# gsw4869/CUDA_LDPC

Measured on AMD Instinct MI355X. Metric: decoded codewords/sec (50-iter flooding min-sum, fixed iterations), higher is better.
Workload: dtype f32; 1 GPU; J4_L24_Z96 rate-0.833 batch=65536 codewords/GPU 50 iters Es/N0=3.0dB; kernel=qc_lds_halfrow-local<nf2,J4,L24,Z96,wc20,wv4,g4,w6>t768_lds79904, frames_per_gpu=65536

## Files before the change

### cuda_ldpc_amd/csrc/bldpc_qc2_body.inc

```
template <typename GM, bool HIST> __global__ __launch_bounds__(GM::TPB, GM::MINW) void QC2_NAME(QcArgs a)
{
    constexpr int NF = GM::NF, L = GM::L, Z = GM::Z, WC = GM::WC, WV = GM::WV, GJ = GM::GJ, ZB = GM::ZB, WCH = GM::WCH;
    constexpr int RPT = GM::RPT, CPT = GM::CPT, NCG = GM::NCG, MSG = GM::MSG;
    static_assert(NF == 2, "the half-row kernel carries a frame pair per lane");
    constexpr bool LOC = GM::LOC;
    constexpr int NL = LOC ? CPT : 0;
    extern __shared__ __attribute__((aligned(16))) char lds[];
    const int chunk = (a.nWG + 7) >> 3;
#if QC2_PERSIST
    const int xcd = (int)(blockIdx.x & 7);
    int wg = 0;
#else
    const int wg = (int)(blockIdx.x & 7) * chunk + (int)(blockIdx.x >> 3);
    if (wg >= a.nWG) return;
#endif

    const int F = a.F;
    const int tid = threadIdx.x;
    const int wave = tid >> 6, lane = tid & 63, h = lane >> 5;
    const int jq = wave / ZB, t = (wave - jq * ZB) * 32 + (lane & 31);
    const int cg = jq * 2 + h;
#if QC2_PERSIST
    int f0 = 0;
#else
    const int f0 = wg * NF;
#endif
    int *lds_flag = reinterpret_cast<int *>(lds + GM::flag_byte);

    const int rbase = ((jq * WC + h * WCH) * Z + t) * MSG;
    const int sbase = (GM::Sslot + cg * Z + t) * MSG;
    int saddr[RPT][WCH];
    v2f32 Rr[RPT][WCH];
    int e0v[RPT], wrv[RPT];
#pragma unroll
    for (int rr = 0; rr < RPT; rr++) {
        e0v[rr] = a.rowptr[jq + rr * GJ];
        wrv[rr] = a.rowptr[jq + rr * GJ + 1] - e0v[rr];
    }
    int wcv[CPT];
#pragma unroll
    for (int cc = 0; cc < CPT; cc++) wcv[cc] = LOC ? 0 : a.wv[cg + cc * NCG];
    int sst[LOC ? CPT : 1];
    int cl[LOC ? CPT : 1];
#pragma unroll
    for (int rr = 0; rr < RPT; rr++) {
        QcCnEdge ed[WCH];
#pragma unroll
        for (int i = 0; i < WCH; i++) ed[i] = a.cn_edges[e0v[rr] + min(h * WCH + i, wrv[rr] - 1)];
#pragma unroll
        for (int i = 0; i < WCH; i++) {
            int c = t + ed[i].shift;
            c = (c >= Z) ? c - Z : c;
            const int slot = (h * WCH + i < wrv[rr]) ? GM::Sslot + ed[i].col * Z + c : GM::inf_slot;
            saddr[rr][i] = slot * MSG;
            if constexpr (LOC) {
                if (i < NL) {
                    sst[i] = slot * MSG;
                    cl[i] = c;
                }
            }
#if !QC2_PERSIST
            Rr[rr][i] = v2f32{0.0f, 0.0f};
            lds_st2(rbase + (rr * GJ * WC + i) * Z * MSG, Rr[rr][i]);
#endif
        }
    }
    v2f32 yreg[CPT];
    int raddr[CPT][WV];
    auto y_load = [&](int cc) -> v2f32 {
        const int n = LOC ? sst[LOC ? cc : 0] / MSG - GM::Sslot : (cg + cc * NCG) * Z + t;
        return a.y_raw ? *reinterpret_cast<const v2f32 *>(a.y_raw + (size_t)n * F + f0)
                       : *reinterpret_cast<const v2f32 *>(a.y + ((size_t)wg * (L * Z) + n) * NF);
    };
#pragma unroll
    for (int cc = 0; cc < CPT; cc++) {
        const int l = cg + cc * NCG;
        if constexpr (LOC) {
            QcVnEdge ed[WV - 1];
#pragma unroll
            for (int kk = 0; kk < WV - 1; kk++) ed[kk] = a.vn_edges[l * WV + kk + (kk >= jq ? 1 : 0)];
#if !QC2_PERSIST
            yreg[cc] = y_load(cc);
#endif
#pragma unroll
            for (int kk = 0; kk < WV - 1; kk++) {
                int r = cl[cc] - ed[kk].shift;
                r = (r < 0) ? r + Z : r;
                raddr[cc][kk] = ((ed[kk].e != 0xffffu) ? ed[kk].e * Z + r : GM::zero_slot) * MSG;
            }
        } else {
        QcVnEdge ed[WV];
#pragma unroll
        for (int k = 0; k < WV; k++) ed[k] = a.vn_edges[l * WV + min(k, wcv[cc] - 1)];
#if !QC2_PERSIST
        yreg[cc] = y_load(cc);
#endif
#pragma unroll
        for (int k = 0; k < WV; k++) {
            int r = t - ed[k].shift;
            r = (r < 0) ? r + Z : r;
            raddr[cc][k] = ((k < wcv[cc]) ? ed[k].e * Z + r : GM::zero_slot) * MSG;
        }
        }
    }
    if (tid < NF) {
        reinterpret_cast<float *>(lds)[GM::zero_slot * NF + tid] = 0.0f;
        reinterpret_cast<float *>(lds)[GM::inf_slot * NF + tid] = __builtin_inff();
        lds_flag[tid] = 0;
        lds_flag[NF + tid] = 0;
    }
    unsigned long long hist = 0;
    unsigned done = 0;
    constexpr unsigned ALL = (1u << NF) - 1u;
#ifdef QC_STAMPS
    int nst = 0;
    auto stamp = [&](unsigned long long v) { if (tid == 0 && nst < QC_STAMPS) a.stamps[(size_t)wg * QC_STAMPS + nst++] = v; };
    const unsigned hwid = __builtin_amdgcn_s_getreg((31 << 11) | 4), xcc = __builtin_amdgcn_s_getreg((31 << 11) | 20);
    stamp(((unsigned long long)xcc << 32) | hwid);
    stamp(__builtin_amdgcn_s_memtime());
    if (a.stagger && ((hwid >> 16) & 1))
        for (int i = 0; i < a.stagger; i += 64 * 16) __builtin_amdgcn_s_sleep(16);
#endif
#if !QC2_PERSIST
    __syncthreads();
#endif
#ifdef QC_STAMPS
    stamp(__builtin_amdgcn_s_memtime());
#endif

    auto vn_phase = [&](bool (&bad)[NF]) {
        constexpr int CB = (CPT * WV <= 12) ? CPT : 1;
        static_for<CPT / CB>([&](auto C0) {
            constexpr int c0 = decltype(C0)::value * CB;
            v2f32 R[CB][WV];
#pragma unroll
            for (int ci = 0; ci < CB; ci++)
#pragma unroll
                for (int k = 0; k < WV; k++) R[ci][k] = lds_ld2(raddr[c0 + ci][k]);
            static_for<CB>([&](auto CI) {
                constexpr int ci = decltype(CI)::value, cc = c0 + ci;
                v2f32 S = v2f32{0.0f, 0.0f};
#pragma unroll
                for (int k = 0; k < WV; k++) S = S + R[ci][k];
                S = S + yreg[cc];
                lds_st2_imm<cc * NCG * Z * MSG>(sbase, S);
                if (HIST) {
                    const bool in_len = ((cg + cc * NCG) * Z + t) < a.length;
                    bad[0] = bad[0] || (in_len && S.x < 0);
                    bad[1] = bad[1] || (in_len && S.y < 0);
                }
            });
            if (CB < CPT) __builtin_amdgcn_sched_barrier(0);
        });
        asm volatile("s_waitcnt lgkmcnt(0)" ::: "memory");
    };
    v2f32 Sloc[LOC ? CPT : 1];
    const int jqs = __builtin_amdgcn_readfirstlane(jq);
    auto vn_phase_loc = [&](auto JJ, bool (&bad)[NF]) {
        constexpr int jj = decltype(JJ)::value;
        v2f32 R[CPT][WV - 1];
#pragma unroll
        for (int cc = 0; cc < CPT; cc++)
#pragma unroll
            for (int kk = 0; kk < WV - 1; kk++) R[cc][kk] = lds_ld2(raddr[cc][kk]);
        static_for<CPT>([&](auto CC) {
            constexpr int cc = decltype(CC)::value;
            v2f32 S = v2f32{0.0f, 0.0f};
            static_for<WV>([&](auto K) {
                constexpr int k = decltype(K)::value;
                if constexpr (k == jj) S = S + Rr[0][cc];
                else S = S + R[cc][k - (k > jj ? 1 : 0)];
            });
            S = S + yreg[cc];
            Sloc[LOC ? cc : 0] = S;
            lds_st2_imm<0>(sst[LOC ? cc : 0], S);
            if (HIST) {
                const bool in_len = (sst[LOC ? cc : 0] / MSG - GM::Sslot) < a.length;
                bad[0] = bad[0] || (in_len && S.x < 0);
                bad[1] = bad[1] || (in_len && S.y < 0);
            }
        });
        asm volatile("s_waitcnt lgkmcnt(0)" ::: "memory");
    };
    auto vn_any = [&](bool (&bad)[NF]) {
        if constexpr (LOC) static_for<GM::J>([&](auto JJ) { if (jqs == decltype(JJ)::value) vn_phase_loc(JJ, bad); });
        else vn_phase(bad);
    };
    auto flags_publish = [&](const bool (&bad)[NF], int it) {
#pragma unroll
        for (int v = 0; v < NF; v++)
            if (bad[v]) lds_flag[(it & 1) * NF + v] = 1;
    };
    auto flags_collect = [&](int it) -> int {
        int flag = 0;
        if (tid < NF) {
            flag = lds_flag[(it & 1) * NF + tid] ? 0 : 1;
            lds_flag[((it + 1) & 1) * NF + tid] = 0;
            if (flag && it <= 64) hist |= (1ull << (it - 1));
        }
        return flag;
    };
    auto emit = [&](unsigned mask, bool (&bad)[NF]) {
        unsigned *obits = a.bits;
        float *oapp = a.app;
        asm volatile("" : "+s"(obits), "+s"(oapp));
#pragma unroll
        for (int cc = 0; cc < CPT; cc++) {
            const int n = (cg + cc * NCG) * Z + t;
            float S[NF];
            lds_ld<NF>(S, lds, sbase + cc * NCG * Z * MSG);
#pragma unroll
            for (int v = 0; v < NF; v++) {
                if (HIST && !((mask >> v) & 1u)) continue;
                const bool neg = S[v] < 0;
                if (!HIST) bad[v] = bad[v] || (n < a.length && neg);
                const unsigned long long m = __ballot(neg);
                if ((tid & 31) == 0 && f0 + v < F) obits[(size_t)(f0 + v) * GM::NW + (n >> 5)] = (unsigned)(m >> (tid & 32));
                if (oapp && f0 + v < F) oapp[(size_t)n * F + f0 + v] = S[v];
            }
        }
    };
    auto retire = [&](int it) -> bool {
        unsigned newly = 0;
#pragma unroll
        for (int v = 0; v < NF; v++)
            if (!lds_flag[(it & 1) * NF + v]) newly |= 1u << v;
        newly &= ~done;
        if (newly) {
            bool unused[NF];
            emit(newly, unused);
            if (tid < NF && ((newly >> tid) & 1u) && f0 + tid < F) a.iters[f0 + tid] = it;
            done |= newly;
        }
        return done == ALL;
    };

#if QC2_PERSIST
    for (;;) {
    if (tid == 0) lds_flag[0] = atomicAdd(&a.work[xcd], 1);
    __syncthreads();
    {
        const int ord = __builtin_amdgcn_readfirstlane(lds_flag[0]);
        if (ord >= chunk || xcd * chunk + ord >= a.nWG) break;
        wg = xcd * chunk + ord;
    }
    __syncthreads();
    f0 = wg * NF;
#pragma unroll
    for (int rr = 0; rr < RPT; rr++)
#pragma unroll
        for (int i = 0; i < WCH; i++) {
            Rr[rr][i] = v2f32{0.0f, 0.0f};
            lds_st2(rbase + (rr * GJ * WC + i) * Z * MSG, Rr[rr][i]);
        }
#pragma unroll
    for (int cc = 0; cc < CPT; cc++) {
        yreg[cc] = y_load(cc);
    }
    if (tid < NF) {
        lds_flag[tid] = 0;
        lds_flag[NF + tid] = 0;
    }
    hist = 0;
    done = 0;
    __syncthreads();
#endif
    auto iterate = [&](auto JJ) {
    for (int it = 1; it < a.max_iter; it++) {
        bool bad[NF];
#pragma unroll
        for (int v = 0; v < NF; v++) bad[v] = false;
        __builtin_amdgcn_s_setprio(QC_PRIO_VN);
        if constexpr (LOC) vn_phase_loc(JJ, bad);
        else vn_phase(bad);
        if (HIST) flags_publish(bad, it);
        __syncthreads();
        __builtin_amdgcn_s_setprio(QC_PRIO_CN);
#ifdef QC_STAMPS
        stamp(__builtin_amdgcn_s_memtime());
#endif
        if (HIST) {
            (void)flags_collect(it);
            if (a.per_frame && retire(it)) return;
        }

#pragma unroll
        for (int rr = 0; rr < RPT; rr++) {
            CnAcc acc[NF];
            {
#ifdef QC2_CHK_SPLIT
                constexpr int CHK = (WCH > 6) ? (WCH + 1) / 2 : WCH;
#else
                constexpr int CHK = (WCH > 6 && !LOC) ? (WCH + 1) / 2 : WCH;
#endif
#pragma unroll
                for (int c0 = 0; c0 < WCH; c0 += CHK) {
                    v2f32 Sv[CHK];
#pragma unroll
                    for (int i = 0; i < CHK && c0 + i < WCH; i++) {
                        if (LOC && c0 + i < NL) Sv[i] = Sloc[LOC ? c0 + i : 0];
                        else Sv[i] = lds_ld2(saddr[rr][c0 + i]);
                    }
#pragma unroll
                    for (int i = 0; i < CHK && c0 + i < WCH; i++) Rr[rr][c0 + i] = Sv[i] - Rr[rr][c0 + i];
                    if (c0 + CHK < WCH) __builtin_amdgcn_sched_barrier(0);
                }
            }
#if QC_ACC_RUNNING
#pragma unroll
            for (int v = 0; v < NF; v++) acc[v].init();
#pragma unroll
            for (int i = 0; i < WCH; i++) {
                acc[0].add(Rr[rr][i].x);
                acc[1].add(Rr[rr][i].y);
            }
#else
            cn_two_smallest<WCH, 2>(reinterpret_cast<const float *>(&Rr[rr][0]), acc[0].m1, acc[0].m2, acc[0].sgn);
            cn_two_smallest<WCH, 2>(reinterpret_cast<const float *>(&Rr[rr][0]) + 1, acc[1].m1, acc[1].m2, acc[1].sgn);
#endif
            uint32_t a1 = f2u(acc[0].m1), b1 = f2u(acc[1].m1), a2 = f2u(acc[0].m2), b2 = f2u(acc[1].m2), as = acc[0].sgn, bs = acc[1].sgn;
            swap32(a1, b1);
            swap32(a2, b2);
            swap32(as, bs);
            const uint32_t m1 = min(a1, b1);
            uint32_t m2u = min(min(max(a1, b1), a2), b2);
            uint32_t keyu = __builtin_amdgcn_bitop3_b32(m1, m2u, __builtin_amdgcn_bitop3_b32(as, bs, 0x80000000u, 0x28), 0x96);
            uint32_t m2v = m2u, keyv = keyu;
            swap32(m2u, m2v);
            swap32(keyu, keyv);
            const float m2f[NF] = {u2f(m2u), u2f(m2v)};
            const uint32_t key[NF] = {keyu, keyv};
            __builtin_amdgcn_s_setprio(LOC ? QC_PRIO_WR_LOC : QC_PRIO_WR);
            static_for<RPT * WCH>([&](auto I) {
                constexpr int r_ = decltype(I)::value / WCH, i = decltype(I)::value % WCH;
                if (r_ != rr) return;
                v2f32 Rn;
                Rn.x = cn_out(Rr[rr][i].x, m2f[0], key[0]);
                Rn.y = cn_out(Rr[rr][i].y, m2f[1], key[1]);
                Rr[rr][i] = Rn;
                if constexpr (!(LOC && i < NL)) lds_st2_imm<(r_ * GJ * WC + i) * Z * MSG>(rbase, Rn);
            });
        }
        asm volatile("s_waitcnt lgkmcnt(0)" ::: "memory");
        __syncthreads();
#ifdef QC_STAMPS
        stamp(__builtin_amdgcn_s_memtime());
#endif
    }
    };
    if constexpr (LOC) static_for<GM::J>([&](auto JJ) { if (jqs == decltype(JJ)::value) iterate(JJ); });
    else iterate(std::integral_constant<int, 0>{});

    int flag = 0;
    if (!(HIST && done == ALL)) {
        bool bad[NF];
#pragma unroll
        for (int v = 0; v < NF; v++) bad[v] = false;
        vn_any(bad);
        if (LOC) __syncthreads();
        emit(~done, bad);
        flags_publish(bad, a.max_iter);
        __syncthreads();
        flag = flags_collect(a.max_iter);
    }
#ifdef QC_STAMPS
    stamp(__builtin_amdgcn_s_memtime());
#endif
    if (tid < NF && f0 + tid < F) {
        const bool stopped = HIST && ((done >> tid) & 1u);
        a.D[(size_t)L * Z * F + f0 + tid] = stopped ? 1 : flag;
        if (HIST && a.hist) a.hist[f0 + tid] = hist;
        if (HIST && a.per_frame && !stopped) a.iters[f0 + tid] = a.max_iter;
    }
#if QC2_PERSIST
    __syncthreads();
    }
#endif
}
```

### cuda_ldpc_amd/csrc/bldpc_qc_kernel.hpp

```cpp
#pragma once
#include <algorithm>
#include <cstdlib>
#include <string>
#include <utility>
#include <vector>

#include "../../include/bldpc.h"
#include "bldpc_math.hpp"
#include "bldpc_qc_assign.hpp"
#include "bldpc_qcc_kernel.hpp"
#include "common.hpp"

#ifndef QC_PRIO_VN
#define QC_PRIO_VN 1
#define QC_PRIO_CN 0
#define QC_PRIO_WR 1
#endif
#ifndef QC_PRIO_WR_LOC
#define QC_PRIO_WR_LOC 0
#endif

namespace cldpc {


struct QcArgs {
    const float *y;
    const float *y_raw;
    int *D;
    unsigned *bits;
    float *app;
    unsigned long long *hist;
    const QcCnEdge *cn_edges;
    const unsigned short *rowptr;
    const QcVnEdge *vn_edges;
    const unsigned char *wv;
    int F, nWG, max_iter, length;
    const unsigned *cn_meta;
    const unsigned *vn_meta;
    int J, L, WVS;
    int lc;
    int per_frame;
    int *work = nullptr;
    int *iters;
#ifdef QC_STAMPS
    unsigned long long *stamps;
    int stagger;
#endif
};

template <int NF> struct Msg;
template <> struct Msg<1> { using T = float; };
typedef float v2f32 __attribute__((ext_vector_type(2)));
template <> struct Msg<2> { using T = v2f32; };

typedef __attribute__((address_space(3))) char lds_char;
template <int NF> __device__ __forceinline__ void lds_ld(float (&d)[NF], const char *, int byte_off)
{
    typedef __attribute__((address_space(3))) const typename Msg<NF>::T lds_msg;
    typename Msg<NF>::T v = *reinterpret_cast<lds_msg *>(static_cast<unsigned>(byte_off));
    __builtin_memcpy(d, &v, sizeof(v));
}
template <int NF> __device__ __forceinline__ void lds_st(char *, int byte_off, const float (&s)[NF])
{
    typedef __attribute__((address_space(3))) typename Msg<NF>::T lds_msg;
    typename Msg<NF>::T v;
    __builtin_memcpy(&v, s, sizeof(v));
    *reinterpret_cast<lds_msg *>(static_cast<unsigned>(byte_off)) = v;
}

template <int NF_, int J_, int L_, int Z_, int WC_, int WV_, int G_, int MINW_, bool LOC_ = false> struct QcGeom {
    static constexpr int NF = NF_, J = J_, L = L_, Z = Z_, WC = WC_, WV = WV_, G = G_, MINW = MINW_;
    static constexpr bool LOC = LOC_;
    static constexpr int NLR = L / J;
    static_assert(!LOC || (Z % 64 == 0 && L % J == 0 && L / J >= 1 && L / J <= WC_ && WV >= 2), "local edges: wave-uniform groups, L / J columns per row");
    static constexpr int RPT = (J + G - 1) / G, CPT = (L + G - 1) / G, TPB = G * Z;
    static constexpr int MSG = NF * 4;
    static constexpr int Sslot = J * WC * Z;
    static constexpr int zero_slot = Sslot + L * Z;
    static constexpr int inf_slot = zero_slot + 1;
    static constexpr int flag_byte = (inf_slot + 1) * MSG;
    static constexpr int lds_bytes = flag_byte + NF * 8;
    static constexpr int NW = (L * Z) / 32;
    static_assert(TPB % 64 == 0 && TPB <= 1024, "workgroup must be whole waves");
    static_assert(Z % 32 == 0, "half-waves must not straddle a thread group");
    static_assert(J % G == 0 && L % G == 0, "groups must tile the block rows and columns");
    static_assert(inf_slot < 65536, "slot indices are packed into 16 bits");
};

// ... 16 lines not shown
{
    static_assert(OFF >= 0 && OFF < 65536, "ds_write has a 16-bit offset");
    if constexpr (NF == 2) asm volatile("ds_write_b64 %0, %1 offset:%2" : : "v"(base), "v"(v), "n"(OFF) : "memory");
    else asm volatile("ds_write_b32 %0, %1 offset:%2" : : "v"(base), "v"(v), "n"(OFF) : "memory");
}
template <int NF> __device__ __forceinline__ float msg_get(const typename Msg<NF>::T &m, int v)
{
    if constexpr (NF == 2) return v ? m.y : m.x;
    else return m;
}
template <int NF> __device__ __forceinline__ void msg_set(typename Msg<NF>::T &m, int v, float x)
{
    if constexpr (NF == 2) { if (v) m.y = x; else m.x = x; }
    else m = x;
}
template <int... Is, typename Fn> __device__ __forceinline__ void static_for_impl(std::integer_sequence<int, Is...>, Fn &&f)
{
    (f(std::integral_constant<int, Is>{}), ...);
}
template <int N, typename Fn> __device__ __forceinline__ void static_for(Fn &&f) { static_for_impl(std::make_integer_sequence<int, N>{}, f); }

template <int WV> constexpr int qc_kdigit(int code, int cc)
{
    for (int i = 0; i < cc; i++) code /= WV;
    return code % WV;
}
template <int WV, int RPT, int NLR> constexpr bool qc_kcode_sorted(int code)
{
    for (int rr = 0; rr < RPT; rr++)
        for (int pp = 0; pp + 1 < NLR; pp++)
            if (qc_kdigit<WV>(code, rr * NLR + pp) > qc_kdigit<WV>(code, rr * NLR + pp + 1)) return false;
    for (int rr = 0; rr + 1 < RPT; rr++) {
        for (int pp = 0; pp < NLR; pp++) {
            const int a = qc_kdigit<WV>(code, rr * NLR + pp), b = qc_kdigit<WV>(code, (rr + 1) * NLR + pp);
            if (a < b) break;
            if (a > b) return false;
        }
    }
    return true;
}
constexpr int qc_ipow(int b, int e) { return e == 0 ? 1 : b * qc_ipow(b, e - 1); }

#define QC1_NAME k_qc
#define QC1_PERSIST 0
#include "bldpc_qc1_body.inc"
#undef QC1_NAME
#undef QC1_PERSIST
#define QC1_NAME k_qcp
#define QC1_PERSIST 1
#include "bldpc_qc1_body.inc"
#undef QC1_NAME
#undef QC1_PERSIST

template <int NF_, int J_, int L_, int Z_, int WC_, int WV_, int GJ_, int MINW_, bool LOC_ = false> struct QcGeom2 {
    static constexpr int NF = NF_, J = J_, L = L_, Z = Z_, WC = WC_, WV = WV_, GJ = GJ_, MINW = MINW_;
    static constexpr bool LOC = LOC_;
    static constexpr int ZB = Z / 32, WCH = WC / 2, NCG = 2 * GJ;
    static constexpr int RPT = J / GJ, CPT = L / NCG, TPB = GJ * ZB * 64;
    static constexpr int MSG = NF * 4;
    static constexpr int Sslot = J * WC * Z;
    static constexpr int zero_slot = Sslot + L * Z;
    static constexpr int inf_slot = zero_slot + 1;
    static constexpr int flag_byte = (inf_slot + 1) * MSG;
    static constexpr int lds_bytes = flag_byte + NF * 8;
    static constexpr int NW = (L * Z) / 32;
    static_assert(Z % 32 == 0 && WC % 2 == 0, "half-waves own 32 circulant positions and half a row each");
    static_assert(J % GJ == 0 && L % NCG == 0, "groups must tile the block rows and columns");
    static_assert(TPB <= 1024 && inf_slot < 65536, "geometry out of range");
    static_assert(!LOC || (GJ == J && WV == J && L / NCG <= WC / 2 && J <= 4), "local edges: one block row per wave, a column's slot k is block row k");
};

__device__ __forceinline__ void swap32(uint32_t &a, uint32_t &b)
{
    auto r = __builtin_amdgcn_permlane32_swap(a, b, false, false);
    a = r[0];
    b = r[1];
}

typedef __attribute__((address_space(3))) v2f32 lds_v2;
__device__ __forceinline__ v2f32 lds_ld2(int byte_off) { return *reinterpret_cast<const lds_v2 *>(static_cast<unsigned>(byte_off)); }
__device__ __forceinline__ void lds_st2(int byte_off, v2f32 v) { *reinterpret_cast<lds_v2 *>(static_cast<unsigned>(byte_off)) = v; }
template <int OFF> __device__ __forceinline__ void lds_st2_imm(int base, v2f32 v)
{
    static_assert(OFF >= 0 && OFF < 65536, "ds_write_b64 has a 16-bit offset");
    asm volatile("ds_write_b64 %0, %1 offset:%2" : : "v"(base), "v"(v), "n"(OFF) : "memory");
}

#define QC2_NAME k_qc2
#define QC2_PERSIST 0
#include "bldpc_qc2_body.inc"
#undef QC2_NAME
#undef QC2_PERSIST
#define QC2_NAME k_qc2p
#define QC2_PERSIST 1
#include "bldpc_qc2_body.inc"
#undef QC2_NAME
#undef QC2_PERSIST

template <int NF> __global__ __launch_bounds__(256) void k_regroup_y(const float *y, float *out, int N, int F)
{
    __shared__ float tile[64][65];
    const int f0 = blockIdx.x * 64, n0 = blockIdx.y * 64;
    const int lane = threadIdx.x & 63, w = threadIdx.x >> 6;
#pragma unroll
    for (int i = 0; i < 16; i++) {
        const int n = n0 + i * 4 + w, f = f0 + lane;
        tile[i * 4 + w][lane] = (n < N && f < F) ? y[(size_t)n * F + f] : 0.0f;
    }
    __syncthreads();
    const int n = n0 + lane;
    for (int q = w; q < 64 / NF; q += 4) {
        const int fg = f0 / NF + q;
        if (n < N && fg * NF < F + NF - 1 && fg < (F + NF - 1) / NF) {
            float v[NF];
#pragma unroll
            for (int k = 0; k < NF; k++) v[k] = tile[lane][q * NF + k];
            typename Msg<NF>::T o;
            __builtin_memcpy(&o, v, sizeof(o));
// ... 290 lines not shown
     k_qcr2<Qcr2Geom<J, L, Z, TPB, WCS, YB, NG>, true>, "regstate-halo", 0, NG, 2, k_qcr2<Qcr2Geom<J, L, Z, TPB, WCS, YB, NG>, true, true>},
    static const QcVariant v[] = {
        X2L(2, 4, 24, 96, 20, 4, 4, 6)
        X2(2, 4, 24, 96, 20, 4, 4, 6)
        X2(2, 8, 24, 96, 10, 6, 4, 6)
        X2(2, 12, 24, 96, 8, 6, 4, 3)
        X2(2, 6, 24, 96, 16, 4, 3, 3)
        X1L(2, 32, 64, 64, 7, 3, 16, 4)
        QC_VARIANTS(X)
        XR(12, 69, 256, 256, 23, 22, 3)
        XR2(4, 24, 512, 512, 20, 8, 5)
        XR(4, 24, 512, 512, 20, 20, 8)
        XC(256, 256, 4, 18, 24)
        XC(160, 192, 5, 12, 24)
        XC(512, 512, 2, 12, 24)
        XC(64, 64, 16, 8, 24)
        XC(96, 128, 8, 12, 24)
        XC(128, 128, 8, 12, 24)
        XC(192, 192, 5, 16, 24)
        XC(320, 320, 3, 24, 24)
        XC(384, 384, 2, 32, 24)
        XC(640, 640, 1, 40, 24)
        XC(1024, 1024, 1, 32, 24)
        XR2(15, 30, 1280, 768, 8, 10, 2)
        XR2(15, 30, 1280, 768, 8, 10, 3)
        XR(15, 30, 1280, 768, 8, 7, 10)
    };
#undef X
#undef X2
#undef X2L
#undef X1L
#undef XC
#undef XR
#undef XR2
    *count = (int)(sizeof(v) / sizeof(v[0]));
    return v;
}

constexpr size_t kLdsBytes = 160 * 1024;
#ifdef QC_STAMPS
static unsigned long long *g_qc_stamps = nullptr;
static int g_qc_stagger = 0;
#endif

struct QcPlan {
    int J = 0, L = 0, Z = 0, nnz = 0, Wc = 0, Wv = 0;
    int variant = -1;
    int frames_per_wg = 0;
    QcCnEdge *d_cn = nullptr;
    unsigned short *d_rowptr = nullptr;
    QcVnEdge *d_vn = nullptr;
    unsigned char *d_wv = nullptr;
    unsigned *d_cn_meta = nullptr, *d_vn_meta = nullptr;
    int WVS = 0, lds_bytes = 0, lc = 0;
    char name[96] = "qc_lds(unavailable)";
    mutable int ran_to_max = 0;
    int persist_grid = 0;
    bool no_persist = false;
    bool force_regroup = false;
    QcPlan *pf = nullptr;
};

struct QcStat {
    int *errs = nullptr;
    int length = 0;
    bool done = false;
};

inline void qc_plan_release(QcPlan *q)
{
    if (q->d_cn) (void)hipFree(q->d_cn);
    if (q->d_rowptr) (void)hipFree(q->d_rowptr);
    if (q->d_vn) (void)hipFree(q->d_vn);
    if (q->d_wv) (void)hipFree(q->d_wv);
    if (q->d_cn_meta) (void)hipFree(q->d_cn_meta);
    if (q->d_vn_meta) (void)hipFree(q->d_vn_meta);
    q->d_cn_meta = nullptr; q->d_vn_meta = nullptr;
    q->d_cn = nullptr; q->d_rowptr = nullptr; q->d_vn = nullptr; q->d_wv = nullptr;
    q->frames_per_wg = 0;
    if (q->pf) {
        qc_plan_release(q->pf);
        delete q->pf;
        q->pf = nullptr;
    }
}

inline int qc_plan_build(QcPlan *q, int J, int L, int Z, const int *H, bool plain = false)
{
    q->J = J; q->L = L; q->Z = Z;
    std::vector<QcCnEdge> cn;
    std::vector<unsigned short> rowptr(J + 1, 0);
    std::vector<int> wv(L, 0);
    int Wc = 0, Wcmin = 1 << 30;
    if (Z > 65535 || L > 65535) return BLDPC_OK;
    for (int j = 0; j < J; j++) {
        for (int l = 0; l < L; l++)
            if (H[j * L + l] != -1) {
                cn.push_back({(unsigned short)l, (unsigned short)H[j * L + l]});
                wv[l]++;
            }
        if (cn.size() > 65535) return BLDPC_OK;
        rowptr[j + 1] = (unsigned short)cn.size();
        Wc = std::max(Wc, (int)(rowptr[j + 1] - rowptr[j]));
        Wcmin = std::min(Wcmin, (int)(rowptr[j + 1] - rowptr[j]));
    }
    const int nnz = (int)cn.size();
    const int Wv = *std::max_element(wv.begin(), wv.end());
    q->nnz = nnz; q->Wc = Wc; q->Wv = Wv;
    int nvar = 0;
    const QcVariant *vars = qc_variants(&nvar);
    const char *pin = getenv("BLDPC_QC_VARIANT");
    const bool no_halo = getenv("BLDPC_NO_HALO") != nullptr;
    q->no_persist = getenv("BLDPC_NO_PERSIST") != nullptr;
    q->force_regroup = getenv("BLDPC_REGROUP") != nullptr;
    const bool no_local = plain || getenv("BLDPC_NO_LOCAL") != nullptr;
    std::vector<int> owner;
    auto qcr2_fits = [&](int ng) -> bool {
        int lc = -1;
        for (int l = 0; l < L && lc < 0; l++)
            if (wv[l] == J) lc = l;
        if (lc < 0 || Z % 64 != 0) return false;
        for (int j = 0; j < J; j++) {
            int rot = 0;
            for (int e = rowptr[j]; e < rowptr[j + 1]; e++)
                if (cn[e].col == lc) rot = cn[e].shift;
            for (int t = 0; t < Z / 64; t++) {
                int nw = 0;
                for (int e = rowptr[j]; e < rowptr[j + 1]; e++)
                    if (cn[e].col != lc && (64 * t + (cn[e].shift - rot + Z) % Z) % Z > Z - 64) nw++;
                if (nw > ng) return false;
            }
        }
        return true;
    };
    for (int vi = 0; vi < nvar && q->variant < 0; vi++) {
        const QcVariant &v = vars[vi];
        if (pin && atoi(pin) != vi) continue;
// ... 124 lines not shown
        rowptr = rowptr2;
    }
    std::vector<int> virt_col(L);
    for (int l = 0; l < L; l++) virt_col[l] = l;
    if (v.loc == 2) {
        const int NLR = L / J, G = v.G;
        std::vector<int> real_of(J);
        for (int j = 0; j < J; j++) real_of[virt_of[j]] = j;
        for (int vj = 0; vj < J; vj++) {
            std::vector<QcCnEdge> loc, oth;
            for (int e = rowptr[vj]; e < rowptr[vj + 1]; e++) (owner[cn[e].col] == real_of[vj] ? loc : oth).push_back(cn[e]);
            auto place = [&](int l) { int o = 0; for (int j2 = 0; j2 < owner[l]; j2++) o += (H[j2 * L + l] != -1) ? 1 : 0; return o; };
            std::stable_sort(loc.begin(), loc.end(), [&](const QcCnEdge &x, const QcCnEdge &y) { return place(x.col) < place(y.col); });
            for (int i = 0; i < NLR; i++) {
                cn[rowptr[vj] + i] = loc[i];
                virt_col[loc[i].col] = (vj % G) + ((vj / G) * NLR + i) * G;
            }
            for (size_t i = 0; i < oth.size(); i++) cn[rowptr[vj] + NLR + i] = oth[i];
        }
    }
    if (v.loc == 1) {
        const int CPT = L / (2 * J), WCH = v.WC / 2;
        std::vector<QcCnEdge> cn2(cn.size());
        for (int j = 0; j < J; j++) {
            std::vector<QcCnEdge> loc, oth;
            for (int e = rowptr[j]; e < rowptr[j + 1]; e++) (owner[cn[e].col] == j ? loc : oth).push_back(cn[e]);
            for (int h = 0; h < 2; h++) {
                QcCnEdge *dst = &cn2[rowptr[j] + h * WCH];
                for (int cc = 0; cc < CPT; cc++) {
                    dst[cc] = loc[h * CPT + cc];
                    virt_col[loc[h * CPT + cc].col] = (2 * j + h) + cc * 2 * J;
                }
                for (int i = CPT; i < WCH; i++) dst[i] = oth[h * (WCH - CPT) + (i - CPT)];
            }
        }
        cn = cn2;
    }
    std::vector<QcVnEdge> vn((size_t)L * vnw, v.loc == 1 ? QcVnEdge{0xffff, 0} : QcVnEdge{0, 0});
    std::vector<int> fill(L, 0), fill_nl(L, 0), kloc(L, 0);
    for (int j = 0; j < J; j++) {
        const int vj = virt_of[j];
        for (int e = rowptr[vj]; e < rowptr[vj + 1]; e++) {
            const int l = cn[e].col;
            if (v.loc == 2) {
                if (owner[l] == j) kloc[virt_col[l]] = fill[l];
                else vn[(size_t)virt_col[l] * v.WV + fill_nl[l]++] = {(unsigned short)(vj * v.WC + (e - rowptr[vj])), cn[e].shift};
                fill[l]++;
            } else if (v.loc == 1) vn[(size_t)virt_col[l] * v.WV + j] = {(unsigned short)(j * v.WC + (e - rowptr[j])), cn[e].shift};
            else if (!generic) vn[(size_t)l * v.WV + fill[l]++] = {(unsigned short)(vj * v.WC + (e - rowptr[vj])), cn[e].shift};
        }
    }
    std::vector<unsigned char> wvb(L);
    for (int l = 0; l < L; l++) wvb[l] = (unsigned char)(v.loc == 2 ? kloc[l] : wv[l]);
    CLDPC_HIP(hipMalloc((void **)&q->d_cn, cn.size() * sizeof(QcCnEdge)), BLDPC_ENOMEM);
    CLDPC_HIP(hipMalloc((void **)&q->d_rowptr, rowptr.size() * sizeof(unsigned short)), BLDPC_ENOMEM);
    CLDPC_HIP(hipMalloc((void **)&q->d_vn, vn.size() * sizeof(QcVnEdge)), BLDPC_ENOMEM);
    CLDPC_HIP(hipMalloc((void **)&q->d_wv, wvb.size()), BLDPC_ENOMEM);
    CLDPC_HIP(hipMemcpy(q->d_cn, cn.data(), cn.size() * sizeof(QcCnEdge), hipMemcpyHostToDevice), BLDPC_EHIP);
    CLDPC_HIP(hipMemcpy(q->d_rowptr, rowptr.data(), rowptr.size() * sizeof(unsigned short), hipMemcpyHostToDevice), BLDPC_EHIP);
    CLDPC_HIP(hipMemcpy(q->d_vn, vn.data(), vn.size() * sizeof(QcVnEdge), hipMemcpyHostToDevice), BLDPC_EHIP);
    CLDPC_HIP(hipMemcpy(q->d_wv, wvb.data(), wvb.size(), hipMemcpyHostToDevice), BLDPC_EHIP);
    CLDPC_HIP(hipFuncSetAttribute((const void *)v.fn, hipFuncAttributeMaxDynamicSharedMemorySize, generic ? (int)kLdsBytes : v.lds_bytes), BLDPC_EHIP);
    CLDPC_HIP(hipFuncSetAttribute((const void *)v.fn_hist, hipFuncAttributeMaxDynamicSharedMemorySize, generic ? (int)kLdsBytes : v.lds_bytes), BLDPC_EHIP);
    if (v.fn_pf) {
        CLDPC_HIP(hipFuncSetAttribute((const void *)v.fn_pf, hipFuncAttributeMaxDynamicSharedMemorySize, generic ? (int)kLdsBytes : v.lds_bytes), BLDPC_EHIP);
        int occ = 0, dev = 0, ncu = 0;
        CLDPC_HIP(hipGetDevice(&dev), BLDPC_EHIP);
        CLDPC_HIP(hipDeviceGetAttribute(&ncu, hipDeviceAttributeMultiprocessorCount, dev), BLDPC_EHIP);
        CLDPC_HIP(hipOccupancyMaxActiveBlocksPerMultiprocessor(&occ, (const void *)v.fn_pf, v.threads, (size_t)q->lds_bytes), BLDPC_EHIP);
        q->persist_grid = std::max(8, ncu * std::max(1, occ) / 8 * 8);
    }
    q->frames_per_wg = v.NF;
    if (v.loc == 2 && !plain && !getenv("BLDPC_LOCAL_PER_FRAME")) {
        q->pf = new QcPlan();
        const int rp = qc_plan_build(q->pf, J, L, Z, H, true);
        if (rp || q->pf->frames_per_wg != v.NF || qc_variants(&nvar)[q->pf->variant].loc) {
            qc_plan_release(q->pf);
            delete q->pf;
            q->pf = nullptr;
            if (rp) return rp;
        }
    }
    snprintf(q->name, sizeof(q->name), "qc_lds_%s<nf%d,J%d,L%d,Z%d,wc%d,wv%d,g%d,w%d>t%d_lds%d", v.tag, v.NF, J, L, v.Z, v.WC, generic ? Wv : v.WV,
             v.G, v.MINW, v.threads, q->lds_bytes);
    return BLDPC_OK;
}

inline bool qc_reads_in_place(const QcPlan *q)
{
    int nvar = 0;
    const QcVariant &v = qc_variants(&nvar)[q->variant];
    return v.NF == 2 && !v.U && !v.regstate;
}

inline int qc_regroup(const QcPlan *q, const float *y, float *yg, int F, hipStream_t st)
{
    int nvar = 0;
    const QcVariant &v = qc_variants(&nvar)[q->variant];
    const int N = q->L * q->Z;
    const dim3 grid((unsigned)((F + 63) / 64), (unsigned)((N + 63) / 64));
    if (v.NF == 2) hipLaunchKernelGGL(k_regroup_y<2>, grid, dim3(256), 0, st, y, yg, N, F);
    else hipLaunchKernelGGL(k_regroup_y<1>, grid, dim3(256), 0, st, y, yg, N, F);
    CLDPC_HIP(hipGetLastError(), BLDPC_EHIP);
    return BLDPC_OK;
}

inline int qc_launch(const QcPlan *q, const float *y, int F, int max_iter, int length, int *D, float *app,
                     unsigned long long *hist, unsigned *bits, hipStream_t st, hipEvent_t ev0 = nullptr, hipEvent_t ev1 = nullptr,
                     int *iters = nullptr, bool expand = true, int *work = nullptr, QcStat *stat = nullptr, bool y_in_place = false)
{
    int nvar = 0;
    const QcVariant &v = qc_variants(&nvar)[q->variant];
    QcArgs a;
    a.y = y; a.y_raw = y_in_place ? y : nullptr; a.D = D; a.bits = bits; a.app = app; a.hist = hist;
    a.per_frame = (iters && hist) ? 1 : 0; a.iters = iters;
    a.cn_edges = q->d_cn; a.rowptr = q->d_rowptr; a.vn_edges = q->d_vn; a.wv = q->d_wv;
    a.F = F;
    a.nWG = (F + q->frames_per_wg - 1) / q->frames_per_wg;
    a.max_iter = max_iter; a.length = length;
    a.cn_meta = q->d_cn_meta; a.vn_meta = q->d_vn_meta; a.J = q->J; a.L = q->L; a.WVS = q->WVS; a.lc = q->lc;
#ifdef QC_STAMPS
    a.stamps = g_qc_stamps; a.stagger = g_qc_stagger;
#endif
    unsigned grid = (unsigned)((a.nWG + 7) / 8 * 8);
    QcKernel fn = hist ? v.fn_hist : v.fn;
    if (a.per_frame && v.fn_pf && work && q->persist_grid > 0 && grid > (unsigned)q->persist_grid && !q->no_persist) {
        CLDPC_HIP(hipMemsetAsync(work, 0, 8 * sizeof(int), st), BLDPC_EHIP);
        a.work = work;
        fn = v.fn_pf;
        grid = (unsigned)q->persist_grid;
    }
    if (ev0) (void)hipEventRecord(ev0, st);
    hipLaunchKernelGGL(fn, dim3(grid), dim3(v.threads), q->lds_bytes, st, a);
    if (ev1) (void)hipEventRecord(ev1, st);
    const int NW = q->L * q->Z / 32;
    if (expand) {
        hipLaunchKernelGGL(k_expand_bits, dim3((unsigned)((F + 1023) / 1024), (unsigned)NW), dim3(256), 0, st, bits, D, F, NW, stat ? stat->errs : nullptr,
                           stat ? stat->length : 0);
        if (stat && stat->errs) stat->done = true;
    }
    CLDPC_HIP(hipGetLastError(), BLDPC_EHIP);
    return BLDPC_OK;
}

inline int qc_decode(const QcPlan *q, const float *y, int F, int max_iter, int length, int exit_mode, int *D, float *app,
                     unsigned long long *flag_hist, unsigned long long *hist_ws, unsigned long long *and_ws, unsigned *bits,
                     float *yg, int *itera, int *iters, int *iters_ws, hipStream_t st, hipEvent_t ev0 = nullptr,
                     hipEvent_t ev1 = nullptr, QcStat *stat = nullptr, const char **used = nullptr)
{
    const QcPlan *qf = q->pf ? q->pf : q;
    if (used) *used = (exit_mode == BLDPC_EXIT_PER_FRAME) ? qf->name : q->name;
    const bool in_place = qc_reads_in_place(q) && (F % 2 == 0) && ((uintptr_t)y % 8 == 0) && !q->force_regroup;
    if (!in_place) {
        int rr = qc_regroup(q, y, yg, F, st);
        if (rr) return rr;
        y = yg;
    }
    if (exit_mode == BLDPC_EXIT_FIXED) {
        *itera = max_iter;
        return qc_launch(q, y, F, max_iter, length, D, app, flag_hist, bits, st, ev0, ev1, nullptr, true, nullptr, stat, in_place);
    }
    if (exit_mode == BLDPC_EXIT_PER_FRAME) {
        *itera = max_iter;
        return qc_launch(qf, y, F, max_iter, length, D, app, flag_hist ? flag_hist : hist_ws, bits, st, ev0, ev1, iters, true, (int *)and_ws, stat, in_place);
    }
    if (max_iter > 64) return fail(BLDPC_EUNSUPPORTED, "QC_LDS with BATCH_GLOBAL exit supports max_iter <= 64 (got %d)", max_iter);
    unsigned long long *hist = flag_hist ? flag_hist : hist_ws;
    auto all_flagged = [&](int iters_run, unsigned long long *all) -> int {
        CLDPC_HIP(hipMemsetAsync(and_ws, 0xFF, sizeof(unsigned long long), st), BLDPC_EHIP);
// ... 39 lines not shown
```

Measured before the change: 13.67 million codewords/s.

## Precompute per-lane LDS address tables on host and peel first iteration

Replaces the kernel prologue's per-thread address computation (rowptr, CN edge and VN edge gathers with modular arithmetic) with a host-built per-lane table, read through coalesced 16-byte loads. It also peels the first decoding iteration: since R messages start at zero, the first VN phase stores only the channel values and the first CN phase skips the subtraction, so the R zero-initialisation stores to LDS are dropped. This adds device memory for the table and a validation step that can disable the variant. The saving is confined to prologue work and one iteration out of fifty, so the effect is probably small.

```diff
diff --git a/cuda_ldpc_amd/csrc/bldpc_qc2_body.inc b/cuda_ldpc_amd/csrc/bldpc_qc2_body.inc
--- a/cuda_ldpc_amd/csrc/bldpc_qc2_body.inc
+++ b/cuda_ldpc_amd/csrc/bldpc_qc2_body.inc
@@ -31,78 +31,37 @@
     const int sbase = (GM::Sslot + cg * Z + t) * MSG;
     int saddr[RPT][WCH];
     v2f32 Rr[RPT][WCH];
-    int e0v[RPT], wrv[RPT];
-#pragma unroll
-    for (int rr = 0; rr < RPT; rr++) {
-        e0v[rr] = a.rowptr[jq + rr * GJ];
-        wrv[rr] = a.rowptr[jq + rr * GJ + 1] - e0v[rr];
-    }
-    int wcv[CPT];
-#pragma unroll
-    for (int cc = 0; cc < CPT; cc++) wcv[cc] = LOC ? 0 : a.wv[cg + cc * NCG];
     int sst[LOC ? CPT : 1];
-    int cl[LOC ? CPT : 1];
-#pragma unroll
-    for (int rr = 0; rr < RPT; rr++) {
-        QcCnEdge ed[WCH];
-#pragma unroll
-        for (int i = 0; i < WCH; i++) ed[i] = a.cn_edges[e0v[rr] + min(h * WCH + i, wrv[rr] - 1)];
-#pragma unroll
-        for (int i = 0; i < WCH; i++) {
-            int c = t + ed[i].shift;
-            c = (c >= Z) ? c - Z : c;
-            const int slot = (h * WCH + i < wrv[rr]) ? GM::Sslot + ed[i].col * Z + c : GM::inf_slot;
-            saddr[rr][i] = slot * MSG;
-            if constexpr (LOC) {
-                if (i < NL) {
-                    sst[i] = slot * MSG;
-                    cl[i] = c;
-                }
-            }
-#if !QC2_PERSIST
-            Rr[rr][i] = v2f32{0.0f, 0.0f};
-            lds_st2(rbase + (rr * GJ * WC + i) * Z * MSG, Rr[rr][i]);
-#endif
-        }
+    int raddr[CPT][WV];
+    {
+        constexpr int NV = LOC ? CPT : 0, WVR = LOC ? WV - 1 : WV;
+        int w[4 * GM::LW];
+#pragma unroll
+        for (int k = 0; k < GM::LW; k++) {
+            const v4i32 x = a.lane[k * GM::TPB + tid];
+            w[4 * k] = x.x; w[4 * k + 1] = x.y; w[4 * k + 2] = x.z; w[4 * k + 3] = x.w;
+        }
+#pragma unroll
+        for (int cc = 0; cc < NV; cc++) sst[LOC ? cc : 0] = (GM::Sslot + w[cc]) * MSG;
+#pragma unroll
+        for (int rr = 0; rr < RPT; rr++)
+#pragma unroll
+            for (int i = 0; i < WCH; i++) saddr[rr][i] = w[NV + rr * WCH + i];
+#pragma unroll
+        for (int cc = 0; cc < CPT; cc++)
+#pragma unroll
+            for (int k = 0; k < WVR; k++) raddr[cc][k] = w[NV + RPT * WCH + cc * WVR + k];
     }
     v2f32 yreg[CPT];
-    int raddr[CPT][WV];
     auto y_load = [&](int cc) -> v2f32 {
         const int n = LOC ? sst[LOC ? cc : 0] / MSG - GM::Sslot : (cg + cc * NCG) * Z + t;
         return a.y_raw ? *reinterpret_cast<const v2f32 *>(a.y_raw + (size_t)n * F + f0)
                        : *reinterpret_cast<const v2f32 *>(a.y + ((size_t)wg * (L * Z) + n) * NF);
     };
-#pragma unroll
-    for (int cc = 0; cc < CPT; cc++) {
-        const int l = cg + cc * NCG;
-        if constexpr (LOC) {
-            QcVnEdge ed[WV - 1];
-#pragma unroll
-            for (int kk = 0; kk < WV - 1; kk++) ed[kk] = a.vn_edges[l * WV + kk + (kk >= jq ? 1 : 0)];
 #if !QC2_PERSIST
-            yreg[cc] = y_load(cc);
-#endif
-#pragma unroll
-            for (int kk = 0; kk < WV - 1; kk++) {
-                int r = cl[cc] - ed[kk].shift;
-                r = (r < 0) ? r + Z : r;
-                raddr[cc][kk] = ((ed[kk].e != 0xffffu) ? ed[kk].e * Z + r : GM::zero_slot) * MSG;
-            }
-        } else {
-        QcVnEdge ed[WV];
-#pragma unroll
-        for (int k = 0; k < WV; k++) ed[k] = a.vn_edges[l * WV + min(k, wcv[cc] - 1)];
-#if !QC2_PERSIST
-        yreg[cc] = y_load(cc);
-#endif
-#pragma unroll
-        for (int k = 0; k < WV; k++) {
-            int r = t - ed[k].shift;
-            r = (r < 0) ? r + Z : r;
-            raddr[cc][k] = ((k < wcv[cc]) ? ed[k].e * Z + r : GM::zero_slot) * MSG;
-        }
-        }
-    }
+#pragma unroll
+    for (int cc = 0; cc < CPT; cc++) yreg[cc] = y_load(cc);
+#endif
     if (tid < NF) {
         reinterpret_cast<float *>(lds)[GM::zero_slot * NF + tid] = 0.0f;
         reinterpret_cast<float *>(lds)[GM::inf_slot * NF + tid] = __builtin_inff();
@@ -182,6 +141,27 @@
         });
         asm volatile("s_waitcnt lgkmcnt(0)" ::: "memory");
     };
+    auto vn_first = [&](bool (&bad)[NF]) {
+        static_for<CPT>([&](auto CC) {
+            constexpr int cc = decltype(CC)::value;
+            const v2f32 S = yreg[cc] + v2f32{0.0f, 0.0f};
+            int n;
+            if constexpr (LOC) {
+                Sloc[LOC ? cc : 0] = S;
+                lds_st2_imm<0>(sst[LOC ? cc : 0], S);
+                n = sst[LOC ? cc : 0] / MSG - GM::Sslot;
+            } else {
+                lds_st2_imm<cc * NCG * Z * MSG>(sbase, S);
+                n = (cg + cc * NCG) * Z + t;
+            }
+            if (HIST) {
+                const bool in_len = n < a.length;
+                bad[0] = bad[0] || (in_len && S.x < 0);
+                bad[1] = bad[1] || (in_len && S.y < 0);
+            }
+        });
+        asm volatile("s_waitcnt lgkmcnt(0)" ::: "memory");
+    };
     auto vn_any = [&](bool (&bad)[NF]) {
         if constexpr (LOC) static_for<GM::J>([&](auto JJ) { if (jqs == decltype(JJ)::value) vn_phase_loc(JJ, bad); });
         else vn_phase(bad);
@@ -247,16 +227,7 @@
     __syncthreads();
     f0 = wg * NF;
 #pragma unroll
-    for (int rr = 0; rr < RPT; rr++)
-#pragma unroll
-        for (int i = 0; i < WCH; i++) {
-            Rr[rr][i] = v2f32{0.0f, 0.0f};
-            lds_st2(rbase + (rr * GJ * WC + i) * Z * MSG, Rr[rr][i]);
-        }
-#pragma unroll
-    for (int cc = 0; cc < CPT; cc++) {
-        yreg[cc] = y_load(cc);
-    }
+    for (int cc = 0; cc < CPT; cc++) yreg[cc] = y_load(cc);
     if (tid < NF) {
         lds_flag[tid] = 0;
         lds_flag[NF + tid] = 0;
@@ -265,13 +236,14 @@
     done = 0;
     __syncthreads();
 #endif
-    auto iterate = [&](auto JJ) {
-    for (int it = 1; it < a.max_iter; it++) {
+    auto iteration = [&](auto JJ, auto FIRST, int it) -> bool {
+        constexpr bool first = decltype(FIRST)::value;
         bool bad[NF];
 #pragma unroll
         for (int v = 0; v < NF; v++) bad[v] = false;
         __builtin_amdgcn_s_setprio(QC_PRIO_VN);
-        if constexpr (LOC) vn_phase_loc(JJ, bad);
+        if constexpr (first) vn_first(bad);
+        else if constexpr (LOC) vn_phase_loc(JJ, bad);
         else vn_phase(bad);
         if (HIST) flags_publish(bad, it);
         __syncthreads();
@@ -281,7 +253,7 @@
 #endif
         if (HIST) {
             (void)flags_collect(it);
-            if (a.per_frame && retire(it)) return;
+            if (a.per_frame && retire(it)) return true;
         }
 
 #pragma unroll
@@ -302,7 +274,7 @@
                         else Sv[i] = lds_ld2(saddr[rr][c0 + i]);
                     }
 #pragma unroll
-                    for (int i = 0; i < CHK && c0 + i < WCH; i++) Rr[rr][c0 + i] = Sv[i] - Rr[rr][c0 + i];
+                    for (int i = 0; i < CHK && c0 + i < WCH; i++) Rr[rr][c0 + i] = first ? Sv[i] : Sv[i] - Rr[rr][c0 + i];
                     if (c0 + CHK < WCH) __builtin_amdgcn_sched_barrier(0);
                 }
             }
@@ -346,17 +318,25 @@
 #ifdef QC_STAMPS
         stamp(__builtin_amdgcn_s_memtime());
 #endif
-    }
-    };
-    if constexpr (LOC) static_for<GM::J>([&](auto JJ) { if (jqs == decltype(JJ)::value) iterate(JJ); });
-    else iterate(std::integral_constant<int, 0>{});
+        return false;
+    };
+    const bool retired = a.max_iter > 1 && iteration(std::integral_constant<int, 0>{}, std::true_type{}, 1);
+    auto iterate = [&](auto JJ) {
+        for (int it = 2; it < a.max_iter; it++)
+            if (iteration(JJ, std::false_type{}, it)) return;
+    };
+    if (!retired) {
+        if constexpr (LOC) static_for<GM::J>([&](auto JJ) { if (jqs == decltype(JJ)::value) iterate(JJ); });
+        else iterate(std::integral_constant<int, 0>{});
+    }
 
     int flag = 0;
     if (!(HIST && done == ALL)) {
         bool bad[NF];
 #pragma unroll
         for (int v = 0; v < NF; v++) bad[v] = false;
-        vn_any(bad);
+        if (a.max_iter > 1) vn_any(bad);
+        else vn_first(bad);
         if (LOC) __syncthreads();
         emit(~done, bad);
         flags_publish(bad, a.max_iter);
diff --git a/cuda_ldpc_amd/csrc/bldpc_qc_kernel.hpp b/cuda_ldpc_amd/csrc/bldpc_qc_kernel.hpp
--- a/cuda_ldpc_amd/csrc/bldpc_qc_kernel.hpp
+++ b/cuda_ldpc_amd/csrc/bldpc_qc_kernel.hpp
@@ -22,6 +22,7 @@
 
 namespace cldpc {
 
+typedef int v4i32 __attribute__((ext_vector_type(4)));
 
 struct QcArgs {
     const float *y;
@@ -34,6 +35,7 @@
     const unsigned short *rowptr;
     const QcVnEdge *vn_edges;
     const unsigned char *wv;
+    const v4i32 *lane;
     int F, nWG, max_iter, length;
     const unsigned *cn_meta;
     const unsigned *vn_meta;
@@ -156,6 +158,10 @@
 #undef QC1_NAME
 #undef QC1_PERSIST
 
+constexpr int qc2_lane_words(int J, int L, int WC, int WV, int GJ, bool loc)
+{
+    return ((loc ? L / (2 * GJ) : 0) + (J / GJ) * (WC / 2) + (L / (2 * GJ)) * (loc ? WV - 1 : WV) + 3) / 4;
+}
 template <int NF_, int J_, int L_, int Z_, int WC_, int WV_, int GJ_, int MINW_, bool LOC_ = false> struct QcGeom2 {
     static constexpr int NF = NF_, J = J_, L = L_, Z = Z_, WC = WC_, WV = WV_, GJ = GJ_, MINW = MINW_;
     static constexpr bool LOC = LOC_;
@@ -168,6 +174,7 @@
     static constexpr int flag_byte = (inf_slot + 1) * MSG;
     static constexpr int lds_bytes = flag_byte + NF * 8;
     static constexpr int NW = (L * Z) / 32;
+    static constexpr int LW = qc2_lane_words(J, L, WC, WV, GJ, LOC);
     static_assert(Z % 32 == 0 && WC % 2 == 0, "half-waves own 32 circulant positions and half a row each");
     static_assert(J % GJ == 0 && L % NCG == 0, "groups must tile the block rows and columns");
     static_assert(TPB <= 1024 && inf_slot < 65536, "geometry out of range");
@@ -564,6 +571,7 @@
     QcVnEdge *d_vn = nullptr;
     unsigned char *d_wv = nullptr;
     unsigned *d_cn_meta = nullptr, *d_vn_meta = nullptr;
+    v4i32 *d_lane = nullptr;
     int WVS = 0, lds_bytes = 0, lc = 0;
     char name[96] = "qc_lds(unavailable)";
     mutable int ran_to_max = 0;
@@ -587,7 +595,8 @@
     if (q->d_wv) (void)hipFree(q->d_wv);
     if (q->d_cn_meta) (void)hipFree(q->d_cn_meta);
     if (q->d_vn_meta) (void)hipFree(q->d_vn_meta);
-    q->d_cn_meta = nullptr; q->d_vn_meta = nullptr;
+    if (q->d_lane) (void)hipFree(q->d_lane);
+    q->d_cn_meta = nullptr; q->d_vn_meta = nullptr; q->d_lane = nullptr;
     q->d_cn = nullptr; q->d_rowptr = nullptr; q->d_vn = nullptr; q->d_wv = nullptr;
     q->frames_per_wg = 0;
     if (q->pf) {
@@ -595,6 +604,59 @@
         delete q->pf;
         q->pf = nullptr;
     }
+}
+
+inline bool qc2_lane_table(const QcVariant &v, const std::vector<unsigned short> &rowptr, const std::vector<QcCnEdge> &cn,
+                           const std::vector<QcVnEdge> &vn, const std::vector<unsigned char> &wvb, std::vector<int> &tab)
+{
+    const bool loc = v.loc == 1;
+    const int Z = v.Z, WC = v.WC, WV = v.WV, GJ = v.G, L = v.L, TPB = v.threads, MSG = v.NF * 4;
+    const int ZB = Z / 32, WCH = WC / 2, NCG = 2 * GJ, RPT = v.J / GJ, CPT = L / NCG, NV = loc ? CPT : 0, WVR = loc ? WV - 1 : WV;
+    const int Sslot = v.J * WC * Z, zero_slot = Sslot + L * Z, inf_slot = zero_slot + 1;
+    const int LW = qc2_lane_words(v.J, L, WC, WV, GJ, loc);
+    tab.assign((size_t)LW * 4 * TPB, 0);
+    bool ok = true;
+    for (int tid = 0; tid < TPB; tid++) {
+        const int wave = tid >> 6, lane = tid & 63, h = lane >> 5;
+        const int jq = wave / ZB, t = (wave - jq * ZB) * 32 + (lane & 31), cg = jq * 2 + h;
+        std::vector<int> w(LW * 4, 0), cl(CPT, 0);
+        for (int rr = 0; rr < RPT; rr++) {
+            const int e0 = rowptr[jq + rr * GJ], wr = rowptr[jq + rr * GJ + 1] - e0;
+            for (int i = 0; i < WCH; i++) {
+                int slot = inf_slot;
+                if (h * WCH + i < wr) {
+                    const QcCnEdge ed = cn[e0 + h * WCH + i];
+                    const int c = (t + ed.shift) % Z;
+                    slot = Sslot + ed.col * Z + c;
+                    if (loc && i < CPT) {
+                        w[i] = ed.col * Z + c;
+                        cl[i] = c;
+                    }
+                }
+                w[NV + rr * WCH + i] = slot * MSG;
+            }
+        }
+        for (int cc = 0; cc < CPT; cc++) {
+            const int l = cg + cc * NCG;
+            for (int k = 0; k < WVR; k++) {
+                int slot = zero_slot;
+                if (loc) {
+                    const QcVnEdge ed = vn[(size_t)l * WV + k + (k >= jq ? 1 : 0)];
+                    if (ed.e != 0xffffu) slot = ed.e * Z + (cl[cc] - ed.shift + Z) % Z;
+                } else if (k < wvb[l]) {
+                    const QcVnEdge ed = vn[(size_t)l * WV + k];
+                    slot = ed.e * Z + (t - ed.shift + Z) % Z;
+                }
+                w[NV + RPT * WCH + cc * WVR + k] = slot * MSG;
+            }
+        }
+        for (int k = 0; k < LW * 4; k++) {
+            const bool var = k < NV, addr = k >= NV && k < NV + RPT * WCH + CPT * WVR;
+            ok = ok && (!var || (w[k] >= 0 && w[k] < L * Z)) && (!addr || (w[k] >= 0 && w[k] < v.lds_bytes - MSG + 1));
+            tab[((size_t)(k / 4) * TPB + tid) * 4 + k % 4] = w[k];
+        }
+    }
+    return ok;
 }
 
 inline int qc_plan_build(QcPlan *q, int J, int L, int Z, const int *H, bool plain = false)
@@ -825,6 +887,12 @@
     }
     std::vector<unsigned char> wvb(L);
     for (int l = 0; l < L; l++) wvb[l] = (unsigned char)(v.loc == 2 ? kloc[l] : wv[l]);
+    if (!generic && std::string(v.tag).compare(0, 7, "halfrow") == 0) {
+        std::vector<int> tab;
+        if (!qc2_lane_table(v, rowptr, cn, vn, wvb, tab)) { q->variant = -1; return BLDPC_OK; }
+        CLDPC_HIP(hipMalloc((void **)&q->d_lane, tab.size() * sizeof(int)), BLDPC_ENOMEM);
+        CLDPC_HIP(hipMemcpy(q->d_lane, tab.data(), tab.size() * sizeof(int), hipMemcpyHostToDevice), BLDPC_EHIP);
+    }
     CLDPC_HIP(hipMalloc((void **)&q->d_cn, cn.size() * sizeof(QcCnEdge)), BLDPC_ENOMEM);
     CLDPC_HIP(hipMalloc((void **)&q->d_rowptr, rowptr.size() * sizeof(unsigned short)), BLDPC_ENOMEM);
     CLDPC_HIP(hipMalloc((void **)&q->d_vn, vn.size() * sizeof(QcVnEdge)), BLDPC_ENOMEM);
@@ -887,7 +955,7 @@
     QcArgs a;
     a.y = y; a.y_raw = y_in_place ? y : nullptr; a.D = D; a.bits = bits; a.app = app; a.hist = hist;
     a.per_frame = (iters && hist) ? 1 : 0; a.iters = iters;
-    a.cn_edges = q->d_cn; a.rowptr = q->d_rowptr; a.vn_edges = q->d_vn; a.wv = q->d_wv;
+    a.cn_edges = q->d_cn; a.rowptr = q->d_rowptr; a.vn_edges = q->d_vn; a.wv = q->d_wv; a.lane = q->d_lane;
     a.F = F;
     a.nWG = (F + q->frames_per_wg - 1) / q->frames_per_wg;
     a.max_iter = max_iter; a.length = length;
```

Measured after the change: 13.92 million codewords/s, median of 6. 1.02x the previous value.
